# 959AI994/Multi-Gate-VAE

Hardware: NVIDIA B200
Metric: gates_per_s_fwd_bwd (higher is better)
Workload: dtype f32

## Files before the change

multi-gate-vae_b200/csrc/mgv_tc.cuh:

```cuda
#pragma once
#include <cuda_fp16.h>
#include "mgv_common.cuh"

namespace tc {

__device__ __forceinline__ uint32_t smem_u32(const void* p) { return (uint32_t)__cvta_generic_to_shared(p); }

__device__ __forceinline__ uint32_t sw128_off(int r, int c16) {
    return (uint32_t)((r >> 3) * 1024 + (r & 7) * 128 + ((c16 ^ (r & 7)) << 4));
}
__device__ __forceinline__ uint32_t plain16_off(int r, int c16) {
    return (uint32_t)((r >> 3) * 256 + c16 * 128 + (r & 7) * 16);
}

__device__ __forceinline__ uint32_t pack_f16x2_sat(float e0, float e1) {
    uint32_t r;
    asm("cvt.rn.satfinite.f16x2.f32 %0, %1, %2;" : "=r"(r) : "f"(e1), "f"(e0));
    return r;
}
__device__ __forceinline__ void split2(float a, float b, uint32_t& hi, uint32_t& lo) {
    hi = pack_f16x2_sat(a, b);
    const float2 hf = __half22float2(*reinterpret_cast<const __half2*>(&hi));
    lo = pack_f16x2_sat(a - hf.x, b - hf.y);
}
// ... 46 lines not shown
    }
};
__device__ __forceinline__ bool mbar_try_wait(uint32_t bar, uint32_t parity) {
    uint32_t done;
    asm volatile(
        "{\n\t.reg .pred p;\n\t"
        "mbarrier.try_wait.parity.shared::cta.b64 p, [%1], %2;\n\t"
        "selp.b32 %0, 1, 0, p;\n\t}"
        : "=r"(done) : "r"(bar), "r"(parity) : "memory");
    return done != 0u;
}
__device__ __forceinline__ void mbar_wait(uint32_t bar, uint32_t parity) {
    WaitGuard g;
#pragma unroll 1
    while (!mbar_try_wait(bar, parity)) g.tick();
}

__device__ __forceinline__ void mbar_wait_warp(uint32_t bar, uint32_t parity, int lane, unsigned sleep_ns = 64) {
    if (lane == 0) {
        WaitGuard g;
#pragma unroll 1
        while (!mbar_try_wait(bar, parity)) {
            if (sleep_ns) __nanosleep(sleep_ns);
            g.tick();
        }
    }
    __syncwarp();
}
__device__ __forceinline__ void mbar_wait_sleep(uint32_t bar, uint32_t parity, unsigned sleep_ns = 64) {
    WaitGuard g;
#pragma unroll 1
    while (!mbar_try_wait(bar, parity)) {
        __nanosleep(sleep_ns);
        g.tick();
    }
}

__device__ __forceinline__ void mbar_expect_tx(uint32_t bar, uint32_t bytes) {
    asm volatile("{\n\t.reg .b64 st;\n\tmbarrier.arrive.expect_tx.shared::cta.b64 st, [%0], %1;\n\t}" ::"r"(bar), "r"(bytes) : "memory");
}
__device__ __forceinline__ void bulk_g2s(uint32_t dst, const void* src, uint32_t bytes, uint32_t bar) {
    asm volatile("cp.async.bulk.shared::cluster.global.mbarrier::complete_tx::bytes [%0], [%1], %2, [%3];"
                 ::"r"(dst), "l"(src), "r"(bytes), "r"(bar) : "memory");
}

__device__ __forceinline__ void bulk_s2g(void* dst, uint32_t src, uint32_t bytes) {
    asm volatile("cp.async.bulk.global.shared::cta.bulk_group [%0], [%1], %2;" ::"l"(dst), "r"(src), "r"(bytes) : "memory");
}
__device__ __forceinline__ uint64_t l2_policy_evict_first() {
    uint64_t pol;
    asm volatile("createpolicy.fractional.L2::evict_first.b64 %0, 1.0;" : "=l"(pol));
    return pol;
}
__device__ __forceinline__ void bulk_s2g_hint(void* dst, uint32_t src, uint32_t bytes, uint64_t pol) {
    asm volatile("cp.async.bulk.global.shared::cta.bulk_group.L2::cache_hint [%0], [%1], %2, %3;" ::"l"(dst), "r"(src), "r"(bytes), "l"(pol) : "memory");
}
__device__ __forceinline__ void bulk_g2s_hint(uint32_t dst, const void* src, uint32_t bytes, uint32_t bar, uint64_t pol) {
    asm volatile("cp.async.bulk.shared::cluster.global.mbarrier::complete_tx::bytes.L2::cache_hint [%0], [%1], %2, [%3], %4;"
                 ::"r"(dst), "l"(src), "r"(bytes), "r"(bar), "l"(pol) : "memory");
}
__device__ __forceinline__ void stg_v4_hint(void* dst, const uint4& v, uint64_t pol) {
    asm volatile("st.global.L2::cache_hint.v4.b32 [%0], {%1,%2,%3,%4}, %5;" ::"l"(dst), "r"(v.x), "r"(v.y), "r"(v.z), "r"(v.w), "l"(pol) : "memory");
}
__device__ __forceinline__ void bulk_commit() { asm volatile("cp.async.bulk.commit_group;" ::: "memory"); }
__device__ __forceinline__ void bulk_wait_read0() { asm volatile("cp.async.bulk.wait_group.read 0;" ::: "memory"); }
__device__ __forceinline__ void bulk_wait0() { asm volatile("cp.async.bulk.wait_group 0;" ::: "memory"); }
__device__ __forceinline__ void named_bar_sync(int id, int nthreads) {
    asm volatile("bar.sync %0, %1;" ::"r"(id), "r"(nthreads) : "memory");
}
__device__ __forceinline__ void tmem_ld8(uint32_t taddr, float (&v)[8]) {
    uint32_t* r = reinterpret_cast<uint32_t*>(v);
    asm volatile("tcgen05.ld.sync.aligned.32x32b.x8.b32 {%0,%1,%2,%3,%4,%5,%6,%7}, [%8];"
                 : "=r"(r[0]), "=r"(r[1]), "=r"(r[2]), "=r"(r[3]), "=r"(r[4]), "=r"(r[5]), "=r"(r[6]), "=r"(r[7])
                 : "r"(taddr) : "memory");
}

__device__ __forceinline__ void fence_async_smem() { asm volatile("fence.proxy.async.shared::cta;" ::: "memory"); }
__device__ __forceinline__ void fence_before_sync() { asm volatile("tcgen05.fence::before_thread_sync;" ::: "memory"); }
__device__ __forceinline__ void fence_after_sync() { asm volatile("tcgen05.fence::after_thread_sync;" ::: "memory"); }

__device__ __forceinline__ void tmem_alloc(uint32_t* slot, uint32_t ncols) {
    asm volatile("tcgen05.alloc.cta_group::1.sync.aligned.shared::cta.b32 [%0], %1;" ::"r"(smem_u32(slot)), "r"(ncols) : "memory");
    asm volatile("tcgen05.relinquish_alloc_permit.cta_group::1.sync.aligned;" ::: "memory");
}
__device__ __forceinline__ void tmem_dealloc(uint32_t base, uint32_t ncols) {
    asm volatile("tcgen05.dealloc.cta_group::1.sync.aligned.b32 %0, %1;" ::"r"(base), "r"(ncols) : "memory");
}
__device__ __forceinline__ void tmem_ld32(uint32_t taddr, float (&v)[32]) {
    uint32_t* r = reinterpret_cast<uint32_t*>(v);
    asm volatile(
        "tcgen05.ld.sync.aligned.32x32b.x32.b32 "
        "{%0,%1,%2,%3,%4,%5,%6,%7,%8,%9,%10,%11,%12,%13,%14,%15,"
        "%16,%17,%18,%19,%20,%21,%22,%23,%24,%25,%26,%27,%28,%29,%30,%31}, [%32];"
        : "=r"(r[0]), "=r"(r[1]), "=r"(r[2]), "=r"(r[3]), "=r"(r[4]), "=r"(r[5]), "=r"(r[6]), "=r"(r[7]),
          "=r"(r[8]), "=r"(r[9]), "=r"(r[10]), "=r"(r[11]), "=r"(r[12]), "=r"(r[13]), "=r"(r[14]), "=r"(r[15]),
          "=r"(r[16]), "=r"(r[17]), "=r"(r[18]), "=r"(r[19]), "=r"(r[20]), "=r"(r[21]), "=r"(r[22]), "=r"(r[23]),
          "=r"(r[24]), "=r"(r[25]), "=r"(r[26]), "=r"(r[27]), "=r"(r[28]), "=r"(r[29]), "=r"(r[30]), "=r"(r[31])
        : "r"(taddr) : "memory");
}
__device__ __forceinline__ void tmem_ld16(uint32_t taddr, float (&v)[16]) {
    uint32_t* r = reinterpret_cast<uint32_t*>(v);
    asm volatile(
        "tcgen05.ld.sync.aligned.32x32b.x16.b32 "
        "{%0,%1,%2,%3,%4,%5,%6,%7,%8,%9,%10,%11,%12,%13,%14,%15}, [%16];"
        : "=r"(r[0]), "=r"(r[1]), "=r"(r[2]), "=r"(r[3]), "=r"(r[4]), "=r"(r[5]), "=r"(r[6]), "=r"(r[7]),
          "=r"(r[8]), "=r"(r[9]), "=r"(r[10]), "=r"(r[11]), "=r"(r[12]), "=r"(r[13]), "=r"(r[14]), "=r"(r[15])
// ... 131 lines not shown
```

multi-gate-vae_b200/csrc/struct_bwd_tc.cu:

```cuda
#include <stdlib.h>
#include <string.h>
#include "struct_layout.cuh"

long long* mgv_debug_trace();
size_t mgv_struct_image_bytes(int num_enc);
int mgv_struct_build_image(const float* weights, int num_enc, uint8_t* image, int precision, cudaStream_t st);
int mgv_struct_bwd_legacy_grid(void);
size_t mgv_struct_bwd_legacy_workspace_bytes(int64_t N, int32_t num_enc);
int mgv_struct_encoder_bwd_legacy(const mgv_schedule* sch, int32_t num_enc, int32_t rounds, int32_t layernorm,
                                  int32_t feat, const float* x, const float* weights, const float* states,
                                  const float* gout, float* grads, void* ws, size_t ws_bytes, int32_t precision,
                                  mgv_stream_t stream);

namespace {
using namespace struct_layout;

constexpr int SGRAD = MGV_STRUCT_GRAD_FLOATS;
constexpr int EPI_WARPS = 8, GATHER_WARPS = 8;
constexpr int THREADS = (EPI_WARPS + GATHER_WARPS + 1) * 32;
constexpr int LDGS = 68;
constexpr uint32_t DG_TILE_BYTES = 131072;
constexpr int CHUNK_TILES_DEFAULT = 2048;

constexpr uint32_t S_G = A_X_LO + 4096;
constexpr uint32_t S_LN = S_G + TM * LDGS * 4;
constexpr uint32_t S_AMAX = S_LN + 512;
constexpr uint32_t S_EX = S_AMAX + 16;
constexpr uint32_t S_BAR = S_EX + 4 * 2 * TM * 4;
constexpr uint32_t S_TMEM = S_BAR + 128;
constexpr uint32_t P_SMEM = S_TMEM + 64 + 1024;
static_assert(P_SMEM <= 227 * 1024, "struct backward: shared memory");
static_assert(A_TILE_BYTES + TM * LDGS * 4 >= TM * 132 * 4, "LayerNorm gradient scratch aliases the tile + staging");
constexpr uint32_t T_ACC = 0, T_OUT = 256, T_LNP = 384;

struct BwdTC {
    int N, feat, layernorm, first, last, dir;
    int tile_beg, tile_end;
    const int* ptr;
    const int* idx;
    const int* order;
    const int* gdesc;
    const unsigned* tile_cost;
    const float* x;
    const uint8_t* image;
    const float* gout;
    const float* in_part; const float* in_agg;
    float* out_part; float* out_agg;
    const uint8_t* tiles;
    size_t tiles_enc_stride;
    uint8_t* dgbuf;
    float* scales;
    unsigned* smin;
    float* partial;
    int gxp;
    int chunk_cap;
    long long* trace;
};
#define PTRACE_MAX(slot) do { if (p.trace && it < 16) atomicMax(reinterpret_cast<unsigned long long*>(p.trace) + (((size_t)blockIdx.y * gridDim.x + blockIdx.x) * 16 + it) * 16 + (slot), (unsigned long long)clock64()); } while (0)
#define PTRACE(slot) do { if (p.trace && it < 16) p.trace[(((size_t)blockIdx.y * gridDim.x + blockIdx.x) * 16 + it) * 16 + (slot)] = clock64(); } while (0)

__device__ __forceinline__ float4 lds4(const float* p) { return *reinterpret_cast<const float4*>(p); }
__device__ __forceinline__ float pow2_scale(float amax) {
    if (!(amax > 0.f) || !isfinite(amax)) return 1.0f;
    const int e = (int)((__float_as_uint(amax) >> 23) & 0xff) - 127;
    int k = 8 - e;
    k = k < -100 ? -100 : (k > 100 ? 100 : k);
    return __uint_as_float((uint32_t)(k + 127) << 23);
}
__device__ __forceinline__ float pow2_scale_keep(float amax, float cur) {
    const float v = amax * cur;
    if (v >= 4.0f && v <= 8192.0f) return cur;
    return (amax > 0.f) ? pow2_scale(amax) : cur;
}

template <bool LOWP>
__global__ void __launch_bounds__(THREADS, 1) struct_bwd_pw_kernel(const BwdTC p) {
    extern __shared__ __align__(1024) uint8_t smem_raw[];
    const uint32_t sbase = (tc::smem_u32(smem_raw) + 1023u) & ~1023u;
    uint8_t* sgen = smem_raw + (sbase - tc::smem_u32(smem_raw));
    const int tid = threadIdx.x, lane = tid & 31, warp = tid >> 5;
    const int enc = blockIdx.y;
    const size_t eoff = (size_t)enc * p.N * D;
    const uint8_t* image = p.image + (size_t)enc * 2 * IMG_BYTES;

    const uint32_t bar_w = sbase + S_BAR, bar_a_full = bar_w + 8, bar_t_full = bar_w + 16, bar_g_empty = bar_w + 24;
    const uint32_t bar_acc_full = bar_w + 32, bar_out_full = bar_w + 40, bar_h_read = bar_w + 48, bar_dg_full = bar_w + 56;
    const uint32_t bar_dg_stored = bar_w + 64;
    uint32_t* tmem_slot = reinterpret_cast<uint32_t*>(sgen + S_TMEM);
    float* s_ln = reinterpret_cast<float*>(sgen + S_LN);
    unsigned* s_amax = reinterpret_cast<unsigned*>(sgen + S_AMAX);
    float* s_g = reinterpret_cast<float*>(sgen + S_G);

    if (tid == 0) {
        tc::mbar_init(bar_w, 1);
        tc::mbar_init(bar_a_full, GATHER_WARPS * 32);
        tc::mbar_init(bar_t_full, 1);
        tc::mbar_init(bar_g_empty, EPI_WARPS * 32);
        tc::mbar_init(bar_acc_full, 1);
        tc::mbar_init(bar_out_full, 1);
        tc::mbar_init(bar_h_read, EPI_WARPS * 32);
        tc::mbar_init(bar_dg_full, EPI_WARPS * 32);
        tc::mbar_init(bar_dg_stored, EPI_WARPS * 32);
        tc::fence_barrier_init();
        tc::mbar_expect_tx(bar_w, IMG_W);
#pragma unroll 1
        for (uint32_t o = 0; o < IMG_W; o += 16384u) tc::bulk_g2s(sbase + o, image + o, 16384u, bar_w);
    }
    if (tid < 2 * D) s_ln[tid] = __ldg(reinterpret_cast<const float*>(image + IMG_W) + tid);
    if (tid < 4) s_amax[tid] = 0u;
    if (warp == 0) tc::tmem_alloc(tmem_slot, 512);
    const int tile_beg = p.tile_beg + (int)blockIdx.x, tile_end = p.tile_end, tile_step = (int)gridDim.x;
    tc::fence_before_sync();
    __syncthreads();
    tc::fence_after_sync();
    const uint32_t tmem = *tmem_slot;

    if (warp >= EPI_WARPS && warp < EPI_WARPS + GATHER_WARPS) {
        const int gw = warp - EPI_WARPS, rg = lane >> 3, c = lane & 7;
        const int4* gdesc = reinterpret_cast<const int4*>(p.gdesc);
        const float* gsrc = p.last ? p.gout + eoff : p.in_part + eoff;
        const float* asrc = p.in_agg + eoff;
        const bool nbg = !p.last;
        int4 dn[4];
#pragma unroll
        for (int ps = 0; ps < 4; ++ps) {
            const int r = tile_beg * TM + gw * 16 + ps * 4 + rg;
            dn[ps] = (tile_beg < tile_end && r < p.N) ? __ldg(gdesc + r) : make_int4(-1, 0, 0, 0);
        }
        int it = 0;
        for (int tile = tile_beg; tile < tile_end; tile += tile_step, ++it) {
            if (lane == 0) PTRACE_MAX(13);
            int4 dc[4];
#pragma unroll
            for (int ps = 0; ps < 4; ++ps) dc[ps] = dn[ps];
#pragma unroll
            for (int ps = 0; ps < 4; ++ps) {
                const int r = (tile + tile_step) * TM + gw * 16 + ps * 4 + rg;
                dn[ps] = (tile + tile_step < tile_end && r < p.N) ? __ldg(gdesc + r) : make_int4(-1, 0, 0, 0);
            }
#pragma unroll
            for (int hf = 0; hf < 2; ++hf) {
                int node[2], beg[2], cnt[2], jn[2];
                float4 g[2][2], va[2][2];
                int maxc = 0;
                const float4 z4 = make_float4(0.f, 0.f, 0.f, 0.f);
#pragma unroll
                for (int q = 0; q < 2; ++q) {
                    const int4 d = dc[2 * hf + q];
                    node[q] = d.x; beg[q] = d.y; cnt[q] = nbg ? d.z : 0; jn[q] = d.w;
                    maxc = max(maxc, cnt[q]);
                    g[q][0] = z4; g[q][1] = z4; va[q][0] = z4; va[q][1] = z4;
                    if (node[q] >= 0) {
                        g[q][0] = mgv_ld4(gsrc + (size_t)node[q] * D + c * 8);
                        g[q][1] = mgv_ld4(gsrc + (size_t)node[q] * D + c * 8 + 4);
                    }
                    if (cnt[q] > 0) {
                        va[q][0] = mgv_ld4(asrc + (size_t)jn[q] * D + c * 8);
                        va[q][1] = mgv_ld4(asrc + (size_t)jn[q] * D + c * 8 + 4);
                    }
                    if (cnt[q] > 1) jn[q] = p.idx[beg[q] + 1] & NODE_MASK;
                }
                float ag[2][8];
#pragma unroll
                for (int q = 0; q < 2; ++q) {
                    ag[q][0] = g[q][0].x + va[q][0].x; ag[q][1] = g[q][0].y + va[q][0].y; ag[q][2] = g[q][0].z + va[q][0].z; ag[q][3] = g[q][0].w + va[q][0].w;
                    ag[q][4] = g[q][1].x + va[q][1].x; ag[q][5] = g[q][1].y + va[q][1].y; ag[q][6] = g[q][1].z + va[q][1].z; ag[q][7] = g[q][1].w + va[q][1].w;
                }
                for (int sl = 1; sl < maxc; sl += 2) {
// ... 28 lines not shown
                    tc::mbar_wait_warp(bar_g_empty, (uint32_t)((it & 1) ^ 1), lane, 64);
                }
#pragma unroll
                for (int q = 0; q < 2; ++q) {
                    float* dst = s_g + (gw * 16 + (2 * hf + q) * 4 + rg) * LDGS + c * 8;
                    *reinterpret_cast<float4*>(dst) = make_float4(ag[q][0], ag[q][1], ag[q][2], ag[q][3]);
                    *reinterpret_cast<float4*>(dst + 4) = make_float4(ag[q][4], ag[q][5], ag[q][6], ag[q][7]);
                }
            }
            tc::mbar_arrive(bar_a_full);
            if (lane == 0) PTRACE_MAX(15);
        }
    } else if (warp == EPI_WARPS + GATHER_WARPS) {
        if (lane == 0 && tile_beg < tile_end) {
            auto load_tile = [&](int t) {
                const uint8_t* src = p.tiles + (size_t)enc * p.tiles_enc_stride + (size_t)t * A_TILE_BYTES;
                if (LOWP) {
                    tc::mbar_expect_tx(bar_t_full, 36864u);
#pragma unroll 1
                    for (uint32_t o = 0; o < 16384u; o += 8192u) {
                        tc::bulk_g2s(sbase + A_AGG_HI + o, src + o, 8192u, bar_t_full);
                        tc::bulk_g2s(sbase + A_H_HI + o, src + (A_H_HI - A_AGG_HI) + o, 8192u, bar_t_full);
                    }
                    tc::bulk_g2s(sbase + A_X_HI, src + (A_X_HI - A_AGG_HI), 4096u, bar_t_full);
                } else {
                    tc::mbar_expect_tx(bar_t_full, A_TILE_BYTES);
#pragma unroll 1
                    for (uint32_t o = 0; o < A_TILE_BYTES; o += 8192u) tc::bulk_g2s(sbase + A_AGG_HI + o, src + o, 8192u, bar_t_full);
                }
            };
            auto issue_recompute = [&](uint32_t tph) {
                tc::mbar_wait_sleep(bar_t_full, tph, 32);
                tc::fence_after_sync();
                const uint32_t d = tmem + T_ACC;
                tc::mma3p<LOWP>(d, tc::desc_k_plain16(sbase + A_X_HI), tc::desc_k_plain16(sbase + A_X_LO),
                         tc::desc_k_plain16(sbase + WX_HI), tc::desc_k_plain16(sbase + WX_LO), tc::make_idesc(128, 256, false, false, LOWP), 0u);
#pragma unroll
                for (int j = 0; j < 4; ++j)
                    tc::mma3p<LOWP>(d, tc::desc_k_sw128(sbase + A_H_HI + 32 * j), tc::desc_k_sw128(sbase + A_H_LO + 32 * j),
                             tc::desc_k_sw128(sbase + WHH_HI + 32 * j), tc::desc_k_sw128(sbase + WHH_LO + 32 * j),
                             tc::make_idesc(128, 128, false, false, LOWP), 1u);
#pragma unroll
                for (int j = 0; j < 4; ++j)
                    tc::mma3p<LOWP>(d + 192u, tc::desc_k_sw128(sbase + A_H_HI + 32 * j), tc::desc_k_sw128(sbase + A_H_LO + 32 * j),
                             tc::desc_k_sw128(sbase + WHH_HI + 16384 + 32 * j), tc::desc_k_sw128(sbase + WHH_LO + 16384 + 32 * j),
                             tc::make_idesc(128, 64, false, false, LOWP), 1u);
#pragma unroll
                for (int j = 0; j < 4; ++j)
                    tc::mma3p<LOWP>(d, tc::desc_k_sw128(sbase + A_AGG_HI + 32 * j), tc::desc_k_sw128(sbase + A_AGG_LO + 32 * j),
                             tc::desc_k_sw128(sbase + WC_HI + 32 * j), tc::desc_k_sw128(sbase + WC_LO + 32 * j),
                             tc::make_idesc(128, 192, false, false, LOWP), 1u);
                tc::mma_commit(bar_acc_full);
            };
            tc::mbar_wait_sleep(bar_w, 0u);
            load_tile(tile_beg);
            issue_recompute(0u);
            int it = 0;
            for (int tile = tile_beg; tile < tile_end; tile += tile_step, ++it) {
                const uint32_t ph = (uint32_t)(it & 1);
                tc::mbar_wait_sleep(bar_acc_full, ph, 32);
                tc::mbar_wait_sleep(bar_h_read, ph, 32);
                if (tile + tile_step < tile_end) load_tile(tile + tile_step);
                tc::mbar_wait_sleep(bar_dg_full, ph, 32);
                tc::fence_after_sync();
                PTRACE(7);
                if (!p.first) {
                    const uint32_t o = tmem + T_OUT;
                    const uint32_t i128 = tc::make_idesc(128, 128, false, true, LOWP), i64 = tc::make_idesc(128, 64, false, true, LOWP);
#pragma unroll
                    for (int s = 0; s < 8; ++s) {
                        const uint32_t a = tmem + T_ACC + 16u * s;
                        tc::mma3p_ts<LOWP>(o, a, a + 8u, tc::desc_mn_sw128(sbase + WC_HI + 2048u * s, WHH_HI - WC_HI),
                                            tc::desc_mn_sw128(sbase + WC_LO + 2048u * s, WHH_LO - WC_LO), i128, 1u);
                    }
#pragma unroll
                    for (int s = 8; s < 12; ++s) {
                        const uint32_t a = tmem + T_ACC + 16u * s;
                        tc::mma3p_ts<LOWP>(o, a, a + 8u, tc::desc_mn_sw128(sbase + WC_HI + 2048u * s, 0),
                                            tc::desc_mn_sw128(sbase + WC_LO + 2048u * s, 0), i64, 1u);
                    }
#pragma unroll
                    for (int s = 12; s < 16; ++s) {
                        const uint32_t a = tmem + T_ACC + 16u * s;
                        tc::mma3p_ts<LOWP>(o + 64u, a, a + 8u, tc::desc_mn_sw128(sbase + WHH_HI + 2048u * (s - 4), 0),
                                            tc::desc_mn_sw128(sbase + WHH_LO + 2048u * (s - 4), 0), i64, 1u);
                    }
                    tc::mma_commit(bar_out_full);
                }
                if (tile + tile_step < tile_end) {
                    tc::mbar_wait_sleep(bar_dg_stored, ph, 32);
                    issue_recompute(ph ^ 1u);
                }
                PTRACE(3);
            }
        }
    } else if (warp < EPI_WARPS) {
        const int wg = warp >> 2, row = (warp & 3) * 32 + lane, u0 = 32 * wg;
        const uint32_t tl = tmem + ((uint32_t)((warp & 3) * 32) << 16);
        const uint32_t t_acc = tl + T_ACC, t_out = tl + T_OUT, t_lnp = tl + T_LNP;
        const float* gs = s_g + row * LDGS;
        float* s_ex = reinterpret_cast<float*>(sgen + S_EX);
        constexpr int EPI_T = EPI_WARPS * 32;
#pragma unroll 1
        for (int cc = 0; cc < 32; cc += 4) {
            tc::tmem_st4(t_lnp + u0 + cc, 0.f, 0.f, 0.f, 0.f);
            tc::tmem_st4(t_lnp + 64 + u0 + cc, 0.f, 0.f, 0.f, 0.f);
        }
        tc::tmem_st_wait();
        float run_scale = 1.0f;
        const uint64_t pol_stream = tc::l2_policy_evict_first();
        int it = 0;
        for (int tile = tile_beg; tile < tile_end; tile += tile_step, ++it) {
            const uint32_t ph = (uint32_t)(it & 1);
            const bool valid = tile * TM + row < p.N;
            const int node = valid ? p.order[tile * TM + row] : 0;
            tc::mbar_wait_warp(bar_t_full, ph, lane, 32);
#pragma unroll
            for (int c8 = 0; c8 < 4; ++c8) {
                const uint32_t off = tc::sw128_off(row, 4 * wg + c8);
                const uint4 hi = *reinterpret_cast<const uint4*>(sgen + A_H_HI + off);
                float h[8];
                if (LOWP) {
                    const uint32_t* w = reinterpret_cast<const uint32_t*>(&hi);
#pragma unroll
                    for (int e = 0; e < 4; ++e) { h[2 * e] = __uint_as_float(w[e] << 16); h[2 * e + 1] = __uint_as_float(w[e] & 0xffff0000u); }
                } else {
                    const uint4 lo = *reinterpret_cast<const uint4*>(sgen + A_H_LO + off);
                    const __half2* h2 = reinterpret_cast<const __half2*>(&hi);
                    const __half2* l2 = reinterpret_cast<const __half2*>(&lo);
#pragma unroll
                    for (int e = 0; e < 4; ++e) {
                        const float2 a = __half22float2(h2[e]), bq = __half22float2(l2[e]);
                        h[2 * e] = a.x + bq.x; h[2 * e + 1] = a.y + bq.y;
                    }
                }
                tc::tmem_st8f(t_out + u0 + 8 * c8, h);
            }
            tc::mbar_arrive(bar_h_read);
            tc::mbar_wait_warp(bar_acc_full, ph, lane, 32);
            tc::mbar_wait_warp(bar_a_full, ph, lane, 32);
            tc::fence_after_sync();
            tc::tmem_st_wait();
            if (tid == 0) PTRACE(4);
            float sum = 0.f;
#pragma unroll 1
            for (int c8 = 0; c8 < 4; ++c8) {
                const int u = u0 + 8 * c8;
                float gr[8], gz[8], gi[8], gh[8], h[8];
                tc::tmem_ld8(t_acc + u, gr);
                tc::tmem_ld8(t_acc + 64 + u, gz);
                tc::tmem_ld8(t_acc + 128 + u, gi);
                tc::tmem_ld8(t_acc + 192 + u, gh);
                tc::tmem_ld8(t_out + u, h);
                tc::tmem_ld_wait();
#pragma unroll
                for (int e = 0; e < 8; ++e) {
                    float r, z, n, hn;
                    gru_gates(gr[e], gz[e], gi[e], gh[e], r, z, n, hn);
                    gr[e] = r; gz[e] = z; gi[e] = n;
                    h[e] = fmaf(z, h[e] - n, n);
                    sum += h[e];
                }
                tc::tmem_st8f(t_acc + u, gr);
                tc::tmem_st8f(t_acc + 64 + u, gz);
                tc::tmem_st8f(t_acc + 128 + u, gi);
                tc::tmem_st8f(t_out + 64 + u, h);
            }
            tc::tmem_st_wait();
            float mean = 0.f, rstd = 1.0f, c1 = 0.f, c2 = 0.f;
            if (p.layernorm) {
                s_ex[wg * TM + row] = sum;
                tc::named_bar_sync(1, EPI_T);
                mean = (s_ex[row] + s_ex[TM + row]) * (1.0f / D);
                float var = 0.f;
#pragma unroll 1
                for (int c8 = 0; c8 < 4; ++c8) {
                    const int u = u0 + 8 * c8;
                    float xv[8];
                    tc::tmem_ld8(t_out + 64 + u, xv);
                    const float4 ga = lds4(gs + u), gb = lds4(gs + u + 4);
                    const float4 wa = lds4(s_ln + u), wb = lds4(s_ln + u + 4);
                    const float gw[8] = {ga.x * wa.x, ga.y * wa.y, ga.z * wa.z, ga.w * wa.w, gb.x * wb.x, gb.y * wb.y, gb.z * wb.z, gb.w * wb.w};
                    tc::tmem_ld_wait();
#pragma unroll
                    for (int e = 0; e < 8; ++e) {
                        const float d = xv[e] - mean;
                        var = fmaf(d, d, var);
                        c1 += gw[e];
                        c2 = fmaf(gw[e], d, c2);
                    }
                }
                s_ex[(2 + wg) * TM + row] = var;
                s_ex[(4 + wg) * TM + row] = c1;
                s_ex[(6 + wg) * TM + row] = c2;
                tc::named_bar_sync(1, EPI_T);
                var = s_ex[2 * TM + row] + s_ex[3 * TM + row];
                c1 = s_ex[4 * TM + row] + s_ex[5 * TM + row];
                c2 = s_ex[6 * TM + row] + s_ex[7 * TM + row];
                rstd = rsqrtf(var * (1.0f / D) + LN_EPS);
                c1 *= (1.0f / D);
                c2 *= rstd * (1.0f / D);
            }
            if (tid == 0) PTRACE(5);
            float amax = 0.f;
#pragma unroll 1
            for (int c4 = 0; c4 < 8; ++c4) {
                const int u = u0 + 4 * c4;
                float r[4], z[4], n[4], hn[4], h[4], xv[4], lw[4], lb[4];
                tc::tmem_ld4(t_acc + u, r);
                tc::tmem_ld4(t_acc + 64 + u, z);
                tc::tmem_ld4(t_acc + 128 + u, n);
                tc::tmem_ld4(t_acc + 192 + u, hn);
                tc::tmem_ld4(t_out + u, h);
                tc::tmem_ld4(t_out + 64 + u, xv);
                if (p.layernorm) { tc::tmem_ld4(t_lnp + u, lw); tc::tmem_ld4(t_lnp + 64 + u, lb); }
                const float4 ga = lds4(gs + u), wa = lds4(s_ln + u);
                const float gv[4] = {ga.x, ga.y, ga.z, ga.w};
                const float wv[4] = {wa.x, wa.y, wa.z, wa.w};
                tc::tmem_ld_wait();
#pragma unroll
                for (int e = 0; e < 4; ++e) {
// ... 141 lines not shown
            tc::tmem_ld_wait();
            *reinterpret_cast<float4*>(scratch + row * 132 + col) = make_float4(v[0], v[1], v[2], v[3]);
            *reinterpret_cast<float4*>(scratch + row * 132 + col + 4) = make_float4(v[4], v[5], v[6], v[7]);
        }
    }
    tc::fence_before_sync();
    __syncthreads();
    if (tid < 2 * D && p.layernorm && tile_beg < tile_end) {
        float s = 0.f;
#pragma unroll 8
        for (int r = 0; r < TM; ++r) s += scratch[r * 132 + tid];
        float* part = p.partial + (((size_t)enc * p.gxp + blockIdx.x) * 2 + p.dir) * SGRAD;
        part[O_LNW + tid] += s;
    }
    if (warp == 0) tc::tmem_dealloc(tmem, 512);
}

__device__ __forceinline__ void red_add4(float4* dst, const float4& v) {
    asm volatile("red.global.add.v4.f32 [%0], {%1,%2,%3,%4};" ::"l"(dst), "f"(v.x), "f"(v.y), "f"(v.z), "f"(v.w) : "memory");
}

constexpr int W_THREADS = 6 * 32;
constexpr uint32_t ST_DG_HI = 0, ST_DG_LO = 32768, ST_AGG_HI = 65536, ST_H_HI = 73728, ST_AGG_LO = 81920, ST_H_LO = 90112;
constexpr uint32_t ST_X_HI = 98304, ST_X_LO = 100352, ST_BYTES = 102400;
constexpr uint32_t W_BAR = 2 * ST_BYTES;
constexpr uint32_t W_TMEM = W_BAR + 64;
constexpr uint32_t W_SMEM = W_TMEM + 64 + 1024;
static_assert(W_SMEM <= 227 * 1024, "struct weight gradient: shared memory");

struct WgTC {
    int ntiles;
    int chunk_cap;
    int dir, gxp;
    const uint8_t* tiles;
    size_t tiles_enc_stride;
    int tile_base;
    const uint8_t* dgbuf;
    const float* scales;
    const unsigned* smin;
    float* partial;
    long long* trace;
};
#define WTRACE(slot) do { if (p.trace && i < 16) p.trace[(((size_t)blockIdx.y * gridDim.x + blockIdx.x) * 16 + i) * 16 + (slot)] = clock64(); } while (0)

template <bool LOWP>
__global__ void __launch_bounds__(W_THREADS, 1) struct_bwd_wgrad_kernel(const WgTC p) {
    extern __shared__ __align__(1024) uint8_t smem_raw[];
    const uint32_t sbase = (tc::smem_u32(smem_raw) + 1023u) & ~1023u;
    uint8_t* sgen = smem_raw + (sbase - tc::smem_u32(smem_raw));
    const int tid = threadIdx.x, lane = tid & 31, warp = tid >> 5;
    const int enc = blockIdx.y;
    const uint32_t bar_full = sbase + W_BAR, bar_ready = bar_full + 16, bar_empty = bar_full + 32, bar_done = bar_full + 48;
    uint32_t* tmem_slot = reinterpret_cast<uint32_t*>(sgen + W_TMEM);
    if (tid == 0) {
        for (int s = 0; s < 2; ++s) {
            tc::mbar_init(bar_full + 8 * s, 1);
            tc::mbar_init(bar_ready + 8 * s, 4 * 32);
            tc::mbar_init(bar_empty + 8 * s, 1);
        }
        tc::mbar_init(bar_done, 1);
        tc::fence_barrier_init();
    }
    if (warp == 0) tc::tmem_alloc(tmem_slot, 512);
    tc::fence_before_sync();
    __syncthreads();
    tc::fence_after_sync();
    const uint32_t tmem = *tmem_slot;
    const int tile_beg = (int)((long long)p.ntiles * blockIdx.x / gridDim.x);
    const int tile_end = (int)((long long)p.ntiles * (blockIdx.x + 1) / gridDim.x);
    const int nhalf = 2 * (tile_end - tile_beg);
    const float smin = __uint_as_float(p.smin[enc]);

    if (warp == 0) {
        if (lane == 0) {
            const uint64_t pol = tc::l2_policy_evict_first();
            for (int i = 0; i < nhalf; ++i) {
                const int s = i & 1, tile = tile_beg + (i >> 1), h = i & 1;
                WTRACE(0);
                tc::mbar_wait_sleep(bar_empty + 8 * s, (uint32_t)(((i >> 1) & 1) ^ 1));
                WTRACE(1);
                tc::mbar_expect_tx(bar_full + 8 * s, LOWP ? 51200u : ST_BYTES);
                const uint8_t* dg = p.dgbuf + ((size_t)enc * p.chunk_cap + tile) * DG_TILE_BYTES + (size_t)h * 32768;
                const uint8_t* at = p.tiles + (size_t)enc * p.tiles_enc_stride + (size_t)(p.tile_base + tile) * A_TILE_BYTES;
                const uint32_t st = sbase + (uint32_t)s * ST_BYTES, bar = bar_full + 8 * s;
                tc::bulk_g2s_hint(st + ST_DG_HI, dg, 16384u, bar, pol);
                tc::bulk_g2s_hint(st + ST_DG_HI + 16384u, dg + 16384, 16384u, bar, pol);
                tc::bulk_g2s_hint(st + ST_AGG_HI, at + 0 + h * 8192, 8192u, bar, pol);
                tc::bulk_g2s_hint(st + ST_H_HI, at + 32768 + h * 8192, 8192u, bar, pol);
                tc::bulk_g2s_hint(st + ST_X_HI, at + 65536 + h * 2048, 2048u, bar, pol);
                if (!LOWP) {
                    tc::bulk_g2s_hint(st + ST_DG_LO, dg + 65536, 16384u, bar, pol);
                    tc::bulk_g2s_hint(st + ST_DG_LO + 16384u, dg + 65536 + 16384, 16384u, bar, pol);
                    tc::bulk_g2s_hint(st + ST_AGG_LO, at + 16384 + h * 8192, 8192u, bar, pol);
                    tc::bulk_g2s_hint(st + ST_H_LO, at + 49152 + h * 8192, 8192u, bar, pol);
                    tc::bulk_g2s_hint(st + ST_X_LO, at + 69632 + h * 2048, 2048u, bar, pol);
                }
            }
        }
    } else if (warp == 1) {
        if (lane == 0) {
            const uint32_t i128 = tc::make_idesc(128, 128, true, true, LOWP), i16 = tc::make_idesc(128, 16, true, true, LOWP);
            for (int i = 0; i < nhalf; ++i) {
                const int s = i & 1;
                WTRACE(4);
                tc::mbar_wait_sleep(bar_ready + 8 * s, (uint32_t)((i >> 1) & 1), 32);
                tc::fence_after_sync();
                WTRACE(5);
                const uint32_t st = sbase + (uint32_t)s * ST_BYTES;
#pragma unroll
                for (int j = 0; j < 4; ++j) {
                    const uint32_t acc = (i > 0 || j > 0) ? 1u : 0u;
                    const uint64_t b_hi = tc::desc_mn_sw128(st + ST_AGG_HI + 2048u * j, 8192), b_lo = tc::desc_mn_sw128(st + ST_AGG_LO + 2048u * j, 8192);
                    const uint64_t x_hi = tc::desc_mn_plain16(st + ST_X_HI + 512u * j), x_lo = tc::desc_mn_plain16(st + ST_X_LO + 512u * j);
#pragma unroll
                    for (int g = 0; g < 2; ++g) {
                        const uint64_t a_hi = tc::make_desc(st + ST_DG_HI + 16384u * g + 256u * j, 128, 1024, tc::LAYOUT_NONE);
                        const uint64_t a_lo = tc::make_desc(st + ST_DG_LO + 16384u * g + 256u * j, 128, 1024, tc::LAYOUT_NONE);
                        tc::mma3p<LOWP>(tmem + 160u * g, a_hi, a_lo, b_hi, b_lo, i128, acc);
                        tc::mma3p<LOWP>(tmem + 160u * g + 128u, a_hi, a_lo, x_hi, x_lo, i16, acc);
                    }
                }
                tc::mma_commit(bar_empty + 8 * s);
                WTRACE(6);
            }
            tc::mma_commit(bar_done);
        }
    } else {
        const int t128 = tid - 64;
        for (int i = 0; i < nhalf; ++i) {
            const int s = i & 1, tile = tile_beg + (i >> 1);
            tc::mbar_wait_warp(bar_full + 8 * s, (uint32_t)((i >> 1) & 1), lane, 32);
            if (tid == 64) WTRACE(2);
            const float m = smin / p.scales[(size_t)enc * p.chunk_cap + tile];
            if (!LOWP && m != 1.0f) {
                const __half2 m2 = __float2half2_rn(m);
                uint4* st = reinterpret_cast<uint4*>(sgen + (size_t)s * ST_BYTES);
#pragma unroll 4
                for (int q = t128; q < 65536 / 16; q += 128) {
                    uint4 v = st[q];
                    __half2* h = reinterpret_cast<__half2*>(&v);
                    h[0] = __hmul2(h[0], m2); h[1] = __hmul2(h[1], m2); h[2] = __hmul2(h[2], m2); h[3] = __hmul2(h[3], m2);
                    st[q] = v;
                }
            }
            tc::fence_async_smem();
            tc::mbar_arrive(bar_ready + 8 * s);
            if (tid == 64) WTRACE(3);
        }
        if (nhalf > 0) {
            const int i = 0;
            if (tid == 64) WTRACE(8);
            tc::mbar_wait_warp(bar_done, 0u, lane, 64);
            tc::fence_after_sync();
            if (tid == 64) WTRACE(9);
            const int L = (warp & 3) * 32 + lane;
            const uint32_t tl = tmem + ((uint32_t)((warp & 3) * 32) << 16);
            float* part = p.partial + (((size_t)enc * p.gxp + blockIdx.x) * 2 + p.dir) * SGRAD;
            float* stg = reinterpret_cast<float*>(sgen);
            constexpr int FLD = 148;
            const float un = 1.0f / smin;
#pragma unroll 1
            for (int g = 0; g < 2; ++g)
#pragma unroll 2
                for (int c8 = 0; c8 < 18; ++c8) {
                    float v[8];
                    tc::tmem_ld8(tl + 160u * g + 8 * c8, v);
                    tc::tmem_ld_wait();
                    float* d = stg + (g * 128 + L) * FLD + 8 * c8;
                    *reinterpret_cast<float4*>(d) = make_float4(v[0] * un, v[1] * un, v[2] * un, v[3] * un);
                    *reinterpret_cast<float4*>(d + 4) = make_float4(v[4] * un, v[5] * un, v[6] * un, v[7] * un);
                }
            tc::named_bar_sync(1, 4 * 32);
            float4* part4 = reinterpret_cast<float4*>(part);
            for (int q = t128; q < G3 * 19; q += 128) {
                const int o = q / 19, c4 = q % 19;
                if (c4 < 18) {
                    const int g = o >= 128 ? 1 : 0, col = c4 < 16 ? 4 * c4 : 128 + 4 * (c4 - 16);
                    const float4 v = *reinterpret_cast<const float4*>(stg + (g * 128 + o - 128 * g) * FLD + col);
                    red_add4(part4 + (O_WCX + o * LDC) / 4 + c4, v);
                }
            }
            for (int q = t128; q < G3 * 17; q += 128) {
                const int o = q / 17, c4 = q % 17;
                if (c4 < 16) {
                    const int row = o >= 128 ? 128 + o - 64 : o;
                    const float4 v = *reinterpret_cast<const float4*>(stg + row * FLD + 64 + 4 * c4);
                    red_add4(part4 + (O_WHH + o * LDM) / 4 + c4, v);
                }
            }
            for (int o = t128; o < G3; o += 128) {
                const int rc = o >= 128 ? 128 + o - 128 : o, rh = o >= 128 ? 128 + o - 64 : o;
                atomicAdd(part + O_BC + o, stg[rc * FLD + 136]);
                atomicAdd(part + O_BIH + o, stg[rc * FLD + 137]);
                atomicAdd(part + O_BHH + o, stg[rh * FLD + 137]);
            }
            if (tid == 64) WTRACE(10);
        }
    }
    tc::fence_before_sync();
    __syncthreads();
    if (warp == 0) tc::tmem_dealloc(tmem, 512);
}

__global__ void struct_reduce_tc_kernel(const float* __restrict__ partial, int gxp, float* __restrict__ grads, int num_enc) {
    const size_t total = (size_t)num_enc * 2 * SGRAD;
    const size_t idx = (size_t)blockIdx.x * blockDim.x + threadIdx.x;
    if (idx >= total) return;
    const int enc = (int)(idx / (2 * SGRAD));
    const size_t rem = idx % (2 * (size_t)SGRAD);
    float s = 0.f;
    for (int b = 0; b < gxp; ++b) s += partial[((size_t)enc * gxp + b) * 2 * SGRAD + rem];
    grads[idx] = s;
}

__global__ void fill_u32_kernel(unsigned* p, unsigned v, int n) {
    const int i = blockIdx.x * blockDim.x + threadIdx.x;
    if (i < n) p[i] = v;
}

int sm_count(int* sms) {
    int dev = 0;
    MGV_CUDA(cudaGetDevice(&dev));
    MGV_CUDA(cudaDeviceGetAttribute(sms, cudaDevAttrMultiProcessorCount, dev));
    return MGV_OK;
}

int chunk_tiles() {
    const char* e = getenv("MGV_STRUCT_CHUNK");
    const int v = e ? atoi(e) : 0;
    return v > 0 ? v : CHUNK_TILES_DEFAULT;
}

bool use_legacy(int precision) {
    (void)precision;
    const char* e = getenv("MGV_STRUCT_BWD");
    return e && !strcmp(e, "mma");
}

size_t tc_workspace_bytes(int64_t N, int num_enc) {
    int sms = 148;
    sm_count(&sms);
    const int64_t ntiles = (N + TM - 1) / TM;
    const int CHUNK_TILES = chunk_tiles();
    const int64_t cap = ntiles < CHUNK_TILES ? ntiles : CHUNK_TILES;
    size_t b = mgv_struct_image_bytes(num_enc) + 256;
    b += 4 * mgv_align_up((size_t)num_enc * N * D * 4 + 256, 256);
    b += mgv_align_up((size_t)sms * 2 * SGRAD * 4 + 256, 256);
    b += mgv_align_up((size_t)num_enc * cap * DG_TILE_BYTES + 1024, 1024);
    b += mgv_align_up((size_t)num_enc * cap * 4 + 256, 256);
    const int64_t chunks = (ntiles + CHUNK_TILES - 1) / CHUNK_TILES;
    b += mgv_align_up((size_t)(chunks > 0 ? chunks : 1) * 2 * 4 + 256, 256) + 4096;
    return b;
}

}

extern "C" int mgv_struct_bwd_grid(void) { return mgv_struct_bwd_legacy_grid(); }

extern "C" size_t mgv_struct_bwd_workspace_bytes(int64_t N, int32_t num_enc) {
    const size_t a = mgv_struct_bwd_legacy_workspace_bytes(N, num_enc), b = tc_workspace_bytes(N, num_enc);
    return a > b ? a : b;
}

extern "C" int mgv_struct_encoder_bwd(const mgv_schedule* sch, int32_t num_enc, int32_t rounds, int32_t layernorm,
                                      int32_t feat, const float* x, const float* weights, const float* states,
                                      const void* tiles, const float* gout, float* grads, void* ws, size_t ws_bytes,
                                      int32_t precision, mgv_stream_t stream) {
    if (use_legacy(precision))
        return mgv_struct_encoder_bwd_legacy(sch, num_enc, rounds, layernorm, feat, x, weights, states, gout, grads, ws, ws_bytes,
                                             precision, stream);
    cudaStream_t st = (cudaStream_t)stream;
    MGV_REQUIRE(sch != nullptr, "struct encoder: null schedule");
    MGV_REQUIRE(num_enc >= 1 && num_enc <= 2, "struct encoder: num_enc must be 1 or 2");
    MGV_REQUIRE(rounds >= 1, "struct encoder: rounds must be >= 1");
    MGV_REQUIRE(feat >= 0 && feat <= MGV_MAX_FEAT, "struct encoder: dim_feature %d > %d", feat, MGV_MAX_FEAT);
    const int N = sch->N;
    MGV_CUDA(cudaMemsetAsync(grads, 0, (size_t)num_enc * 2 * SGRAD * sizeof(float), st));
    if (N == 0) return MGV_OK;
    MGV_REQUIRE(sch->deg_order_in && sch->deg_order_out && sch->tile_cost_in && sch->tile_cost_out && sch->gdesc_in && sch->gdesc_out,
                "struct encoder: the schedule carries no degree order (mgv_build_degree_order)");
    MGV_REQUIRE(tiles != nullptr, "mgv_struct_encoder_bwd: the operand tiles saved by mgv_struct_encoder_fwd are required (tiles == NULL)");
    if (ws_bytes < mgv_struct_bwd_workspace_bytes(N, num_enc)) {
        mgv_set_error("mgv_struct_encoder_bwd: workspace %zu < %zu bytes", ws_bytes, mgv_struct_bwd_workspace_bytes(N, num_enc));
        return MGV_ERR_WORKSPACE;
    }
    int sms = 0;
    int rc = sm_count(&sms);
    if (rc != MGV_OK) return rc;
    const int ntiles = (N + TM - 1) / TM;
    const int CHUNK_TILES = chunk_tiles();
    const int cap = ntiles < CHUNK_TILES ? ntiles : CHUNK_TILES;
    const int chunks = (ntiles + CHUNK_TILES - 1) / CHUNK_TILES;
    const int gxp = sms / num_enc > 0 ? sms / num_enc : 1;
    const int steps = 2 * rounds;
    const size_t slot = (size_t)N * D;
    (void)states;

    MgvArena a(ws, ws_bytes);
    uint8_t* image = a.take<uint8_t>((size_t)num_enc * 2 * IMG_BYTES);
    float* part[2];
    float* agg[2];
    part[0] = a.take<float>((size_t)num_enc * slot); part[1] = a.take<float>((size_t)num_enc * slot);
    agg[0] = a.take<float>((size_t)num_enc * slot); agg[1] = a.take<float>((size_t)num_enc * slot);
    float* partial = a.take<float>((size_t)num_enc * gxp * 2 * SGRAD);
    a.off = mgv_align_up(a.off, 1024);
    uint8_t* dgbuf = a.take<uint8_t>((size_t)num_enc * cap * DG_TILE_BYTES);
    float* scales = a.take<float>((size_t)num_enc * cap);
    unsigned* smin = a.take<unsigned>((size_t)chunks * 2);
    MGV_REQUIRE(a.ok(), "mgv_struct_encoder_bwd: workspace layout overflow");
    MGV_REQUIRE(precision == 0 || precision == 1, "struct encoder: precision must be 0 (fp32-accurate) or 1 (bf16)");
    rc = mgv_struct_build_image(weights, num_enc, image, precision, st);
    if (rc != MGV_OK) return rc;
    MGV_CUDA(cudaMemsetAsync(partial, 0, (size_t)num_enc * gxp * 2 * SGRAD * sizeof(float), st));
    const bool lowp = precision == 1;
    const void* pw_fn = lowp ? (const void*)struct_bwd_pw_kernel<true> : (const void*)struct_bwd_pw_kernel<false>;
    const void* wg_fn = lowp ? (const void*)struct_bwd_wgrad_kernel<true> : (const void*)struct_bwd_wgrad_kernel<false>;
    MGV_CUDA(cudaFuncSetAttribute(pw_fn, cudaFuncAttributeMaxDynamicSharedMemorySize, (int)P_SMEM));
    MGV_CUDA(cudaFuncSetAttribute(wg_fn, cudaFuncAttributeMaxDynamicSharedMemorySize, (int)W_SMEM));

    for (int k = steps; k >= 1; --k) {
        const int dir = (k & 1) ? 0 : 1;
        fill_u32_kernel<<<(chunks * 2 + 63) / 64, 64, 0, st>>>(smin, 0x7f000000u, chunks * 2);
        mgv_count_launches(1);
        for (int ch = 0; ch < chunks; ++ch) {
            const int tb = ch * CHUNK_TILES, te = (tb + CHUNK_TILES < ntiles) ? tb + CHUNK_TILES : ntiles;
            int gx = gxp;
            if (gx > te - tb) gx = te - tb;
            BwdTC p{};
            p.N = N; p.feat = feat; p.layernorm = layernorm; p.first = (k == 1); p.last = (k == steps); p.dir = dir;
            p.tile_beg = tb; p.tile_end = te;
            p.ptr = dir == 0 ? sch->in_ptr : sch->out_ptr;
            p.idx = dir == 0 ? sch->in_src : sch->out_pack;
            p.order = dir == 0 ? sch->deg_order_in : sch->deg_order_out;
            p.gdesc = dir == 0 ? sch->gdesc_in : sch->gdesc_out;
            p.tile_cost = dir == 0 ? sch->tile_cost_in : sch->tile_cost_out;
            p.x = x;
            p.image = image + (size_t)dir * IMG_BYTES;
            p.gout = gout;
            p.in_part = part[k & 1]; p.in_agg = agg[k & 1];
            p.out_part = part[(k - 1) & 1]; p.out_agg = agg[(k - 1) & 1];
            p.tiles = (const uint8_t*)tiles + (size_t)(k - 1) * ntiles * A_TILE_BYTES;
            p.tiles_enc_stride = (size_t)steps * ntiles * A_TILE_BYTES;
            p.dgbuf = dgbuf; p.scales = scales; p.smin = smin + 2 * ch;
            p.partial = partial; p.gxp = gxp; p.chunk_cap = cap;
            p.trace = (k == 2 && ch == 0 && !getenv("MGV_TRACE_WGRAD")) ? mgv_debug_trace() : nullptr;
            if (lowp) struct_bwd_pw_kernel<true><<<dim3(gx, num_enc), THREADS, P_SMEM, st>>>(p);
            else struct_bwd_pw_kernel<false><<<dim3(gx, num_enc), THREADS, P_SMEM, st>>>(p);
            WgTC w{};
            w.ntiles = te - tb; w.chunk_cap = cap; w.dir = dir; w.gxp = gxp;
            w.tiles = p.tiles; w.tiles_enc_stride = p.tiles_enc_stride; w.tile_base = tb;
            w.dgbuf = dgbuf; w.scales = scales; w.smin = smin + 2 * ch; w.partial = partial;
            w.trace = (k == 2 && ch == 0 && getenv("MGV_TRACE_WGRAD")) ? mgv_debug_trace() : nullptr;
            if (lowp) struct_bwd_wgrad_kernel<true><<<dim3(gx, num_enc), W_THREADS, W_SMEM, st>>>(w);
            else struct_bwd_wgrad_kernel<false><<<dim3(gx, num_enc), W_THREADS, W_SMEM, st>>>(w);
            mgv_count_launches(2);
        }
    }
    const size_t total = (size_t)num_enc * 2 * SGRAD;
    struct_reduce_tc_kernel<<<(unsigned)((total + 255) / 256), 256, 0, st>>>(partial, gxp, grads, num_enc);
    mgv_count_launches(1);
    return mgv_check_cuda(cudaGetLastError(), "mgv_struct_encoder_bwd");
}
```

Baseline: 19.06 million.

## Chain backward kernels with programmatic dependent launch and double-buffer smin reset

Launches the pointwise and weight-gradient backward kernels with programmatic stream serialization. Each kernel signals dependents early and waits only before it consumes prior results, so setup work (barrier init, TMEM allocation, weight loads, recompute MMAs) overlaps the tail of the previous kernel. The per-step fill kernel is replaced by double-buffered smin slots, with the next buffer reset inside the pointwise kernel. The weight-gradient epilogue also batches TMEM loads into 16-wide groups. This adds ordering subtleties: correctness now depends on the placement of griddepcontrol.wait relative to reads of the previous kernel's outputs.

```diff
diff --git a/multi-gate-vae_b200/csrc/mgv_tc.cuh b/multi-gate-vae_b200/csrc/mgv_tc.cuh
--- a/multi-gate-vae_b200/csrc/mgv_tc.cuh
+++ b/multi-gate-vae_b200/csrc/mgv_tc.cuh
@@ -122,6 +122,8 @@
     asm volatile("createpolicy.fractional.L2::evict_first.b64 %0, 1.0;" : "=l"(pol));
     return pol;
 }
+__device__ __forceinline__ void grid_dep_launch() { asm volatile("griddepcontrol.launch_dependents;" ::: "memory"); }
+__device__ __forceinline__ void grid_dep_wait() { asm volatile("griddepcontrol.wait;" ::: "memory"); }
 __device__ __forceinline__ void bulk_s2g_hint(void* dst, uint32_t src, uint32_t bytes, uint64_t pol) {
     asm volatile("cp.async.bulk.global.shared::cta.bulk_group.L2::cache_hint [%0], [%1], %2, %3;" ::"l"(dst), "r"(src), "r"(bytes), "l"(pol) : "memory");
 }
diff --git a/multi-gate-vae_b200/csrc/struct_bwd_tc.cu b/multi-gate-vae_b200/csrc/struct_bwd_tc.cu
--- a/multi-gate-vae_b200/csrc/struct_bwd_tc.cu
+++ b/multi-gate-vae_b200/csrc/struct_bwd_tc.cu
@@ -21,6 +21,7 @@
 constexpr int LDGS = 68;
 constexpr uint32_t DG_TILE_BYTES = 131072;
 constexpr int CHUNK_TILES_DEFAULT = 2048;
+constexpr unsigned SMIN_INIT = 0x7f000000u;
 
 constexpr uint32_t S_G = A_X_LO + 4096;
 constexpr uint32_t S_LN = S_G + TM * LDGS * 4;
@@ -51,6 +52,8 @@
     uint8_t* dgbuf;
     float* scales;
     unsigned* smin;
+    unsigned* smin_reset;
+    int smin_reset_n;
     float* partial;
     int gxp;
     int chunk_cap;
@@ -90,6 +93,7 @@
     float* s_ln = reinterpret_cast<float*>(sgen + S_LN);
     unsigned* s_amax = reinterpret_cast<unsigned*>(sgen + S_AMAX);
     float* s_g = reinterpret_cast<float*>(sgen + S_G);
+    tc::grid_dep_launch();
 
     if (tid == 0) {
         tc::mbar_init(bar_w, 1);
@@ -114,6 +118,7 @@
     __syncthreads();
     tc::fence_after_sync();
     const uint32_t tmem = *tmem_slot;
+    if (warp >= EPI_WARPS && warp < EPI_WARPS + GATHER_WARPS) tc::grid_dep_wait();
 
     if (warp >= EPI_WARPS && warp < EPI_WARPS + GATHER_WARPS) {
         const int gw = warp - EPI_WARPS, rg = lane >> 3, c = lane & 7;
@@ -248,8 +253,8 @@
                              tc::make_idesc(128, 192, false, false, LOWP), 1u);
                 tc::mma_commit(bar_acc_full);
             };
+            load_tile(tile_beg);
             tc::mbar_wait_sleep(bar_w, 0u);
-            load_tile(tile_beg);
             issue_recompute(0u);
             int it = 0;
             for (int tile = tile_beg; tile < tile_end; tile += tile_step, ++it) {
@@ -334,7 +339,6 @@
             }
             tc::mbar_arrive(bar_h_read);
             tc::mbar_wait_warp(bar_acc_full, ph, lane, 32);
-            tc::mbar_wait_warp(bar_a_full, ph, lane, 32);
             tc::fence_after_sync();
             tc::tmem_st_wait();
             if (tid == 0) PTRACE(4);
@@ -363,6 +367,12 @@
                 tc::tmem_st8f(t_out + 64 + u, h);
             }
             tc::tmem_st_wait();
+            if (it == 0) {
+                tc::grid_dep_wait();
+                if (p.smin_reset && blockIdx.x == 0 && blockIdx.y == 0 && tid == 0)
+                    for (int i = 0; i < p.smin_reset_n; ++i) p.smin_reset[i] = SMIN_INIT;
+            }
+            tc::mbar_wait_warp(bar_a_full, ph, lane, 32);
             float mean = 0.f, rstd = 1.0f, c1 = 0.f, c2 = 0.f;
             if (p.layernorm) {
                 s_ex[wg * TM + row] = sum;
@@ -610,6 +620,7 @@
     const int enc = blockIdx.y;
     const uint32_t bar_full = sbase + W_BAR, bar_ready = bar_full + 16, bar_empty = bar_full + 32, bar_done = bar_full + 48;
     uint32_t* tmem_slot = reinterpret_cast<uint32_t*>(sgen + W_TMEM);
+    tc::grid_dep_launch();
     if (tid == 0) {
         for (int s = 0; s < 2; ++s) {
             tc::mbar_init(bar_full + 8 * s, 1);
@@ -624,6 +635,7 @@
     __syncthreads();
     tc::fence_after_sync();
     const uint32_t tmem = *tmem_slot;
+    tc::grid_dep_wait();
     const int tile_beg = (int)((long long)p.ntiles * blockIdx.x / gridDim.x);
     const int tile_end = (int)((long long)p.ntiles * (blockIdx.x + 1) / gridDim.x);
     const int nhalf = 2 * (tile_end - tile_beg);
@@ -719,14 +731,18 @@
             const float un = 1.0f / smin;
 #pragma unroll 1
             for (int g = 0; g < 2; ++g)
-#pragma unroll 2
-                for (int c8 = 0; c8 < 18; ++c8) {
-                    float v[8];
-                    tc::tmem_ld8(tl + 160u * g + 8 * c8, v);
+#pragma unroll 1
+                for (int c48 = 0; c48 < 3; ++c48) {
+                    float v[3][16];
+#pragma unroll
+                    for (int j = 0; j < 3; ++j) tc::tmem_ld16(tl + 160u * g + 48 * c48 + 16 * j, v[j]);
                     tc::tmem_ld_wait();
-                    float* d = stg + (g * 128 + L) * FLD + 8 * c8;
-                    *reinterpret_cast<float4*>(d) = make_float4(v[0] * un, v[1] * un, v[2] * un, v[3] * un);
-                    *reinterpret_cast<float4*>(d + 4) = make_float4(v[4] * un, v[5] * un, v[6] * un, v[7] * un);
+                    float* d = stg + (g * 128 + L) * FLD + 48 * c48;
+#pragma unroll
+                    for (int j = 0; j < 3; ++j)
+#pragma unroll
+                        for (int e = 0; e < 16; e += 4)
+                            *reinterpret_cast<float4*>(d + 16 * j + e) = make_float4(v[j][e] * un, v[j][e + 1] * un, v[j][e + 2] * un, v[j][e + 3] * un);
                 }
             tc::named_bar_sync(1, 4 * 32);
             float4* part4 = reinterpret_cast<float4*>(part);
@@ -780,6 +796,18 @@
     int dev = 0;
     MGV_CUDA(cudaGetDevice(&dev));
     MGV_CUDA(cudaDeviceGetAttribute(sms, cudaDevAttrMultiProcessorCount, dev));
+    return MGV_OK;
+}
+
+template <typename P>
+int launch_chained(void (*kern)(P), dim3 grid, int threads, uint32_t smem, cudaStream_t st, bool pdl, const P& p) {
+    cudaLaunchAttribute at[1];
+    at[0].id = cudaLaunchAttributeProgrammaticStreamSerialization;
+    at[0].val.programmaticStreamSerializationAllowed = 1;
+    cudaLaunchConfig_t cfg = {};
+    cfg.gridDim = grid; cfg.blockDim = dim3(threads); cfg.dynamicSmemBytes = smem; cfg.stream = st;
+    cfg.attrs = at; cfg.numAttrs = pdl ? 1 : 0;
+    MGV_CUDA(cudaLaunchKernelEx(&cfg, kern, p));
     return MGV_OK;
 }
 
@@ -807,7 +835,7 @@
     b += mgv_align_up((size_t)num_enc * cap * DG_TILE_BYTES + 1024, 1024);
     b += mgv_align_up((size_t)num_enc * cap * 4 + 256, 256);
     const int64_t chunks = (ntiles + CHUNK_TILES - 1) / CHUNK_TILES;
-    b += mgv_align_up((size_t)(chunks > 0 ? chunks : 1) * 2 * 4 + 256, 256) + 4096;
+    b += mgv_align_up((size_t)(chunks > 0 ? chunks : 1) * 4 * 4 + 256, 256) + 4096;
     return b;
 }
 
@@ -864,7 +892,7 @@
     a.off = mgv_align_up(a.off, 1024);
     uint8_t* dgbuf = a.take<uint8_t>((size_t)num_enc * cap * DG_TILE_BYTES);
     float* scales = a.take<float>((size_t)num_enc * cap);
-    unsigned* smin = a.take<unsigned>((size_t)chunks * 2);
+    unsigned* smin = a.take<unsigned>((size_t)chunks * 4);
     MGV_REQUIRE(a.ok(), "mgv_struct_encoder_bwd: workspace layout overflow");
     MGV_REQUIRE(precision == 0 || precision == 1, "struct encoder: precision must be 0 (fp32-accurate) or 1 (bf16)");
     rc = mgv_struct_build_image(weights, num_enc, image, precision, st);
@@ -876,10 +904,12 @@
     MGV_CUDA(cudaFuncSetAttribute(pw_fn, cudaFuncAttributeMaxDynamicSharedMemorySize, (int)P_SMEM));
     MGV_CUDA(cudaFuncSetAttribute(wg_fn, cudaFuncAttributeMaxDynamicSharedMemorySize, (int)W_SMEM));
 
+    fill_u32_kernel<<<(chunks * 4 + 63) / 64, 64, 0, st>>>(smin, SMIN_INIT, chunks * 4);
+    mgv_count_launches(1);
+    bool pdl = false;
     for (int k = steps; k >= 1; --k) {
         const int dir = (k & 1) ? 0 : 1;
-        fill_u32_kernel<<<(chunks * 2 + 63) / 64, 64, 0, st>>>(smin, 0x7f000000u, chunks * 2);
-        mgv_count_launches(1);
+        unsigned* smin_k = smin + (size_t)(k & 1) * chunks * 2;
         for (int ch = 0; ch < chunks; ++ch) {
             const int tb = ch * CHUNK_TILES, te = (tb + CHUNK_TILES < ntiles) ? tb + CHUNK_TILES : ntiles;
             int gx = gxp;
@@ -899,18 +929,21 @@
             p.out_part = part[(k - 1) & 1]; p.out_agg = agg[(k - 1) & 1];
             p.tiles = (const uint8_t*)tiles + (size_t)(k - 1) * ntiles * A_TILE_BYTES;
             p.tiles_enc_stride = (size_t)steps * ntiles * A_TILE_BYTES;
-            p.dgbuf = dgbuf; p.scales = scales; p.smin = smin + 2 * ch;
+            p.dgbuf = dgbuf; p.scales = scales; p.smin = smin_k + 2 * ch;
+            p.smin_reset = (ch == 0 && k > 1) ? smin + (size_t)((k - 1) & 1) * chunks * 2 : nullptr;
+            p.smin_reset_n = chunks * 2;
             p.partial = partial; p.gxp = gxp; p.chunk_cap = cap;
             p.trace = (k == 2 && ch == 0 && !getenv("MGV_TRACE_WGRAD")) ? mgv_debug_trace() : nullptr;
-            if (lowp) struct_bwd_pw_kernel<true><<<dim3(gx, num_enc), THREADS, P_SMEM, st>>>(p);
-            else struct_bwd_pw_kernel<false><<<dim3(gx, num_enc), THREADS, P_SMEM, st>>>(p);
+            rc = launch_chained(lowp ? struct_bwd_pw_kernel<true> : struct_bwd_pw_kernel<false>, dim3(gx, num_enc), THREADS, P_SMEM, st, pdl, p);
+            if (rc != MGV_OK) return rc;
+            pdl = true;
             WgTC w{};
             w.ntiles = te - tb; w.chunk_cap = cap; w.dir = dir; w.gxp = gxp;
             w.tiles = p.tiles; w.tiles_enc_stride = p.tiles_enc_stride; w.tile_base = tb;
-            w.dgbuf = dgbuf; w.scales = scales; w.smin = smin + 2 * ch; w.partial = partial;
+            w.dgbuf = dgbuf; w.scales = scales; w.smin = p.smin; w.partial = partial;
             w.trace = (k == 2 && ch == 0 && getenv("MGV_TRACE_WGRAD")) ? mgv_debug_trace() : nullptr;
-            if (lowp) struct_bwd_wgrad_kernel<true><<<dim3(gx, num_enc), W_THREADS, W_SMEM, st>>>(w);
-            else struct_bwd_wgrad_kernel<false><<<dim3(gx, num_enc), W_THREADS, W_SMEM, st>>>(w);
+            rc = launch_chained(lowp ? struct_bwd_wgrad_kernel<true> : struct_bwd_wgrad_kernel<false>, dim3(gx, num_enc), W_THREADS, W_SMEM, st, true, w);
+            if (rc != MGV_OK) return rc;
             mgv_count_launches(2);
         }
     }
```

Result: faster. 19.51 million (median of 6 runs) (+2.4%).
